# Gilgamesh666666/Point-cloud-registration-based-on-rotation-invariant-feature

Measured on AMD Instinct MI355X. Metric: point-clouds/sec (1024 pts, k=32) PPF+sph-vox forward, higher is better.
Workload: dtype f32; 1 GPU; sph-dg extractor forward: self-KNN k=32 + local PPF + sph-vox r=32^3 + sph-devox + descriptor; clouds_per_gpu=32, points=1024, k=32, resolution=32, channels=64, global_batch=32, parallelism=dp1 (clouds sharded, descriptor all-gather), schedule=6, steps_per_launch=200, distinct_batches=20

## Files before the change

### point-cloud-registration-based-on-rotation-invariant-feature_amd/csrc/knn_wsel.hip

```cpp
#include "knn_spatial.hpp"

namespace pcr {

template <int W>
constexpr int wsel_chunk() { return W == 8 ? 2 : 1; }
static inline bool wsel_narrow(int nblk, int b) { return (size_t)nblk * b * 8 > 4096; }
constexpr int kWselCap = 64;
constexpr int kWselTmax = 0x461C3FFF;

#define PCR_WSEL_VCC_STAGE(NAME, CTRL, LOW)                                        \
  __device__ inline unsigned NAME(unsigned x) {                                    \
    unsigned t;                                                                    \
    asm volatile("s_nop 1\n\t"                                                     \
                 "v_sub_co_u32_dpp %1, vcc, %0, %0 " CTRL " row_mask:0xf bank_mask:0xf\n\t" \
                 "s_xor_b32 vcc_lo, vcc_lo, " LOW "\n\t"                           \
                 "s_xor_b32 vcc_hi, vcc_hi, " LOW "\n\t"                           \
                 "v_cndmask_b32_dpp %0, %0, %0, vcc " CTRL " row_mask:0xf bank_mask:0xf" \
                 : "+v"(x), "=&v"(t)                                               \
                 :                                                                 \
                 : "vcc");                                                         \
    return x;                                                                      \
  }
PCR_WSEL_VCC_STAGE(wsel_x1, "quad_perm:[1,0,3,2]", "0x55555555")
PCR_WSEL_VCC_STAGE(wsel_x2, "quad_perm:[2,3,0,1]", "0x33333333")
PCR_WSEL_VCC_STAGE(wsel_m4, "quad_perm:[3,2,1,0]", "0x33333333")
#undef PCR_WSEL_VCC_STAGE
#define PCR_WSEL_MINMAX_STAGE(NAME, LO, HI, MLO, MHI)                              \
  __device__ inline unsigned NAME(unsigned x) {                                    \
    unsigned a;                                                                    \
    asm volatile("s_nop 1\n\t"                                                     \
                 "v_min_u32_dpp %0, %1, %1 " LO " " MLO "\n\t"                     \
                 "v_max_u32_dpp %0, %1, %1 " HI " " MHI                            \
                 : "=&v"(a)                                                        \
                 : "v"(x));                                                        \
    return a;                                                                      \
  }
PCR_WSEL_MINMAX_STAGE(wsel_m8, "row_half_mirror", "row_half_mirror",
                      "row_mask:0xf bank_mask:0x5", "row_mask:0xf bank_mask:0xa")
PCR_WSEL_MINMAX_STAGE(wsel_m16, "row_mirror", "row_mirror",
                      "row_mask:0xf bank_mask:0x3", "row_mask:0xf bank_mask:0xc")
PCR_WSEL_MINMAX_STAGE(wsel_x4, "row_shl:4", "row_shr:4",
                      "row_mask:0xf bank_mask:0x5", "row_mask:0xf bank_mask:0xa")
PCR_WSEL_MINMAX_STAGE(wsel_x8, "row_shl:8", "row_shr:8",
                      "row_mask:0xf bank_mask:0x3", "row_mask:0xf bank_mask:0xc")
#undef PCR_WSEL_MINMAX_STAGE
#define PCR_WSEL_ROW_STAGE(NAME, FETCH, RLO, RHI)                                  \
  __device__ inline unsigned NAME(unsigned x) {                                    \
    unsigned a, p;                                                                 \
    asm volatile("s_nop 1\n\t" FETCH                                               \
                 "s_nop 1\n\t"                                                     \
                 "v_min_u32_dpp %0, %1, %2 quad_perm:[0,1,2,3] row_mask:" RLO " bank_mask:0xf\n\t" \
                 "v_max_u32_dpp %0, %1, %2 quad_perm:[0,1,2,3] row_mask:" RHI " bank_mask:0xf" \
                 : "=&v"(a), "+v"(x), "=&v"(p)                                     \
                 :);                                                               \
    return a;                                                                      \
  }
PCR_WSEL_ROW_STAGE(wsel_x16,
                   "v_mov_b32_e32 %2, %1\n\t"
                   "s_nop 1\n\t"
                   "v_permlane16_swap_b32 %2, %2\n\t",
                   "0x5", "0xa")
PCR_WSEL_ROW_STAGE(wsel_m32,
                   "v_mov_b32_dpp %2, %1 row_mirror row_mask:0xf bank_mask:0xf\n\t"
                   "s_nop 1\n\t"
                   "v_permlane16_swap_b32 %2, %2\n\t",
                   "0x5", "0xa")
PCR_WSEL_ROW_STAGE(wsel_m64,
                   "v_mov_b32_dpp %2, %1 row_mirror row_mask:0xf bank_mask:0xf\n\t"
                   "s_nop 1\n\t"
                   "v_permlane16_swap_b32 %2, %2\n\t"
                   "s_nop 1\n\t"
                   "v_permlane32_swap_b32 %2, %2\n\t",
                   "0x3", "0xc")
#undef PCR_WSEL_ROW_STAGE

__device__ inline unsigned wsel_sort64(unsigned x) {
  x = wsel_x1(x);
  x = wsel_m4(x);
  x = wsel_x1(x);
  x = wsel_m8(x);
  x = wsel_x2(x);
  x = wsel_x1(x);
  x = wsel_m16(x);
  x = wsel_x4(x);
  x = wsel_x2(x);
  x = wsel_x1(x);
  x = wsel_m32(x);
  x = wsel_x8(x);
  x = wsel_x4(x);
  x = wsel_x2(x);
  x = wsel_x1(x);
  x = wsel_m64(x);
  x = wsel_x16(x);
  x = wsel_x8(x);
  x = wsel_x4(x);
  x = wsel_x2(x);
  x = wsel_x1(x);
  asm volatile("s_nop 1");
  return x;
}

__device__ inline unsigned long long wsel_sort64_exact(unsigned long long x, int lane) {
  for (int kk = 2; kk <= 64; kk <<= 1) {
    for (int jj = kk >> 1; jj > 0; jj >>= 1) {
      const int m = jj == (kk >> 1) ? kk - 1 : jj;
      const unsigned long long p = shfl_xor_u64(x, m);
      const bool lower = (lane & jj) == 0;
      x = lower ? (x < p ? x : p) : (x < p ? p : x);
    }
  }
  return x;
}

__device__ __attribute__((always_inline)) inline void wsel_append(unsigned long long m,
                                                                  unsigned addr, unsigned d,
                                                                  int lane, int r) {
  unsigned t, p;
  unsigned long long save;
  asm volatile("v_add_u32_e32 %0, %2, %1" : "=v"(p) : "v"(lane), "i"(64 * r));
  asm volatile(
      "s_mov_b64 %1, exec\n\t"
      "s_mov_b64 exec, %2\n\t"
      "v_mbcnt_lo_u32_b32 %0, %3, 0\n\t"
      "v_mbcnt_hi_u32_b32 %0, %4, %0\n\t"
      "v_lshl_add_u32 %0, %0, 2, %5\n\t"
      "ds_write2st64_b32 %0, %6, %7 offset1:1\n\t"
      "s_mov_b64 exec, %1"
      : "=&v"(t), "=&s"(save)
      : "s"(m), "s"((unsigned)m), "s"((unsigned)(m >> 32)), "s"(addr), "v"(d), "v"(p)
      : "memory");
}

template <int R, int W>
__global__ __launch_bounds__(W * 64) void knn_wsel_kernel(KnnSet s, int k) {
  constexpr int kWselWaves = W;
  constexpr int kWselChunk = wsel_chunk<W>();
  __shared__ unsigned kbuf_s[kWselWaves][2][kWselCap];
  __shared__ int tile_s[kBlk][kSortedK + 1];
  __shared__ int qnext_s;
  __shared__ __align__(16) float cx_s[R * kBlk], cy_s[R * kBlk], cz_s[R * kBlk];
  __shared__ __align__(16) int cj_s[R * kBlk];
  static_assert(sizeof(kbuf_s[0][0]) == 256, "wsel_append's offset");
  static_assert(sizeof(cx_s) % (64 * 16) == 0, "whole LDS-DMA pieces");
  const int b = blockIdx.y, qblk = blockIdx.x;
  const int wv = __builtin_amdgcn_readfirstlane(threadIdx.x >> 6);
  const int lane = threadIdx.x & 63;
  const size_t cb = (size_t)b * s.npad;
  lds_dma_copy<16>(cx_s, s.x + cb, 4 * s.npad);
  lds_dma_copy<16>(cy_s, s.y + cb, 4 * s.npad);
  lds_dma_copy<16>(cz_s, s.z + cb, 4 * s.npad);
  lds_dma_copy<16>(cj_s, s.j + cb, 4 * s.npad);
  if (threadIdx.x == 0) qnext_s = 0;
  wait_vmcnt<0>();
  __syncthreads();
  if (s.npad < R * kBlk) {
    for (int i = s.npad + threadIdx.x; i < R * kBlk; i += kWselWaves * kBlk) {
      cx_s[i] = cy_s[i] = cz_s[i] = __builtin_nanf("");
      cj_s[i] = -1;
    }
    __syncthreads();
  }
  typedef float pf2v __attribute__((ext_vector_type(2)));
  pf2v cx[R / 2], cy[R / 2], cz[R / 2];
#pragma unroll
  for (int h = 0; h < R / 2; h++) {
    const int p = 2 * h * kBlk + lane;
    cx[h] = pf2v{cx_s[p], cx_s[p + kBlk]};
    cy[h] = pf2v{cy_s[p], cy_s[p + kBlk]};
    cz[h] = pf2v{cz_s[p], cz_s[p + kBlk]};
  }
  const int pq = qblk * kBlk + lane;
  const float qxl = cx_s[pq], qyl = cy_s[pq], qzl = cz_s[pq];
  const int qjl = cj_s[pq];
  auto grab = [&]() {
    int v = 0;
    if (lane == 0)
      v = __hip_atomic_fetch_add(&qnext_s, kWselChunk, __ATOMIC_RELAXED, __HIP_MEMORY_SCOPE_WORKGROUP);
    return v;
  };
  int q0 = __builtin_amdgcn_readfirstlane(grab());
  int tb = kWselTmax;
  if (q0 < kBlk) {
    const float* bx = s.box + ((size_t)b * s.nblk + qblk) * 8;
    const float qx = readlane_f(qxl, q0), qy = readlane_f(qyl, q0), qz = readlane_f(qzl, q0);
    if (min(kBlk, s.n - qblk * kBlk) >= k) {
      const float u = box_ub(qx, qy, qz, bx);
      if (u < PCR_KNN_UNDEF) tb = (int)__float_as_uint(u);
    }
  }
  unsigned* kd = kbuf_s[wv][0];
  int* kj = (int*)kbuf_s[wv][1];
  const unsigned kd_addr =
      (unsigned)(uintptr_t)((__attribute__((address_space(3))) unsigned*)kd);
  const float tgt = 0.5f * (float)(k + kWselCap);
#pragma unroll 1
  for (int qi = q0; qi < kBlk;) {
    const int qj = __builtin_amdgcn_readlane(qjl, qi);
    if (qj < 0) {
      if (lane < kSortedK) tile_s[qi][lane] = 0;
      if (++qi % kWselChunk == 0) qi = __builtin_amdgcn_readfirstlane(grab());
      continue;
    }
    const float qx = readlane_f(qxl, qi), qy = readlane_f(qyl, qi), qz = readlane_f(qzl, qi);
    const pf2v qx2 = {qx, qx}, qy2 = {qy, qy}, qz2 = {qz, qz};
    unsigned db[R];
#pragma unroll
    for (int h = 0; h < R / 2; h++) {
      const pf2v a = qx2 - cx[h], bq = qy2 - cy[h], c = qz2 - cz[h];
      pf2v d = a * a;
      d = __builtin_elementwise_fma(bq, bq, d);
      d = __builtin_elementwise_fma(c, c, d);
      db[2 * h] = __float_as_uint(d[0]);
      db[2 * h + 1] = __float_as_uint(d[1]);
    }
    constexpr bool kKeep = R <= 16;
    unsigned long long msk[kKeep ? R : 1];
    auto count_le = [&](int bits) {
      int pc[4] = {0, 0, 0, 0};
#pragma unroll
      for (int r = 0; r < R; r++) {
        const unsigned long long m = __ballot(db[r] <= (unsigned)bits);
        if (kKeep) msk[kKeep ? r : 0] = m;
        pc[r & 3] += __popcll(m);
      }
      return (pc[0] + pc[1]) + (pc[2] + pc[3]);
    };
    int lo = -1, hi = 0x7F800000, cnt_lo = 0, cnt = 0;
    bool exact = false;
#pragma unroll 1
    for (int pass = 0;; pass++) {
      cnt = count_le(tb);
      if (cnt >= k && cnt <= kWselCap) break;
      if (cnt < k) {
        lo = tb;
        cnt_lo = cnt;
        if (tb >= kWselTmax) break;
      } else {
        hi = tb;
      }
      if (hi - lo <= 1) {
        exact = true;
        break;
      }
      int nb;
      if (pass < 3) {
        const float f = __uint_as_float((unsigned)tb) *
                        __builtin_amdgcn_exp2f(0.6666667f * __builtin_amdgcn_logf(
                                                                tgt * __builtin_amdgcn_rcpf((float)max(cnt, 1))));
        nb = f < 1e30f ? (int)__float_as_uint(f) : kWselTmax;
      } else {
        nb = lo + ((hi - lo) >> 1);
      }
      nb = min(nb, kWselTmax);
      if (nb <= lo || nb >= hi) nb = lo + ((hi - lo) >> 1);
      tb = __builtin_amdgcn_readfirstlane(nb);
    }
    int ntake;
    if (!exact) {
      unsigned addr = kd_addr;
#pragma unroll
      for (int r = 0; r < R; r++) {
        const unsigned long long m = kKeep ? msk[kKeep ? r : 0] : __ballot(db[r] <= (unsigned)tb);
        if (m != 0ull) {
          wsel_append(m, addr, db[r], lane, r);
          addr += 4u * (unsigned)__popcll(m);
        }
      }
      ntake = cnt;
    } else {
      const int need = k - cnt_lo;
      auto cj = [&](int r) { return cj_s[64 * r + lane]; };
      int jl = -1, jh = s.n - 1;
#pragma unroll 1
      while (jh - jl > 1) {
        const int jm = jl + ((jh - jl) >> 1);
        int c = 0;
#pragma unroll
        for (int r = 0; r < R; r++) c += __popcll(__ballot(db[r] == (unsigned)hi && cj(r) <= jm));
        if (c >= need) jh = jm;
        else jl = jm;
      }
      unsigned addr = kd_addr;
#pragma unroll
      for (int r = 0; r < R; r++) {
        const unsigned long long m =
            __ballot(db[r] < (unsigned)hi || (db[r] == (unsigned)hi && cj(r) <= jh));
        if (m != 0ull) {
          wsel_append(m, addr, db[r], lane, r);
          addr += 4u * (unsigned)__popcll(m);
        }
      }
      ntake = k;
    }
    const unsigned dl = lane < ntake ? kd[lane] : 0xFFFFFFFFu;
    unsigned key = lane < ntake ? ((dl >> 6) << 6) | (unsigned)lane : 0x7FFFFFFFu;
    key = wsel_sort64(key);
    const unsigned nxt = (unsigned)__builtin_amdgcn_mov_dpp((int)key, 0x130, 0xF, 0xF, false);
    const bool tie = lane < k && lane + 1 < ntake && (key >> 6) == (nxt >> 6);
    const bool slow = __any(tie);
    if (!slow) {
      const int jo = lane < ntake ? cj_s[kj[key & 63u]] : 0;
      if (lane < k) tile_s[qi][lane] = jo;
    } else {
      unsigned long long skey = ~0ull;
      if (lane < ntake) skey = ((unsigned long long)kd[lane] << 32) | (unsigned)cj_s[kj[lane]];
      skey = wsel_sort64_exact(skey, lane);
      if (lane < k) tile_s[qi][lane] = lane < ntake ? (int)(unsigned)(skey & 0xFFFFFFFFull) : 0;
    }
    __atomic_signal_fence(__ATOMIC_SEQ_CST);
    if (++qi % kWselChunk == 0) qi = __builtin_amdgcn_readfirstlane(grab());
  }
  __syncthreads();
  for (int sl = wv; sl < k; sl += kWselWaves)
    s.sidx[((size_t)b * kSortedK + sl) * s.npad + (size_t)qblk * kBlk + lane] = tile_s[lane][sl];
}

void launch_wsel(const KnnSet& s, int b, int k, hipStream_t st) {
  if (wsel_narrow(s.nblk, b))
    hipLaunchKernelGGL((knn_wsel_kernel<16, 8>), dim3(s.nblk, b), dim3(8 * 64), 0, st, s, k);
  else
    hipLaunchKernelGGL((knn_wsel_kernel<16, 12>), dim3(s.nblk, b), dim3(12 * 64), 0, st, s, k);
}

}
```

Before: 474,400 point-clouds/sec.

## Search KNN threshold on per-lane minima before a full exact-count fallback

The radius-threshold search in the wave-select KNN now runs on each lane's minimum distance (a single ballot per pass) rather than counting every candidate register on each pass. Each step uses a precomputed log-log order-statistic table held in lanes to jump the threshold. Candidates are then appended once with a capacity guard, and the earlier full count/bisect path runs only when the resulting count falls outside [k, cap]. This trims ballot and popcount work per search pass, but adds an extra append pass and a fallback path whenever the lane-minimum estimate misses.

Result: no change. 471,400 point-clouds/sec (-0.6%).

```diff
diff --git a/point-cloud-registration-based-on-rotation-invariant-feature_amd/csrc/knn_wsel.hip b/point-cloud-registration-based-on-rotation-invariant-feature_amd/csrc/knn_wsel.hip
--- a/point-cloud-registration-based-on-rotation-invariant-feature_amd/csrc/knn_wsel.hip
+++ b/point-cloud-registration-based-on-rotation-invariant-feature_amd/csrc/knn_wsel.hip
@@ -7,6 +7,9 @@
 static inline bool wsel_narrow(int nblk, int b) { return (size_t)nblk * b * 8 > 4096; }
 constexpr int kWselCap = 64;
 constexpr int kWselTmax = 0x461C3FFF;
+constexpr int kWselLaneWin = 4;
+constexpr int kWselLaneEst = 5;
+constexpr float kWselLaneInv = 1.0f / 64.5f;
 
 #define PCR_WSEL_VCC_STAGE(NAME, CTRL, LOW)                                        \
   __device__ inline unsigned NAME(unsigned x) {                                    \
@@ -193,6 +196,11 @@
   const unsigned kd_addr =
       (unsigned)(uintptr_t)((__attribute__((address_space(3))) unsigned*)kd);
   const float tgt = 0.5f * (float)(k + kWselCap);
+  auto lane_g = [](float m) {
+    return (int)(5592405.0f * __log2f(-__log2f(1.0f - kWselLaneInv * m)));
+  };
+  const int gtab = lane_g((float)(lane + 1));
+  const int gtgt = __builtin_amdgcn_readfirstlane(lane_g((float)k + 0.5f * (float)kWselLaneWin));
 #pragma unroll 1
   for (int qi = q0; qi < kBlk;) {
     const int qj = __builtin_amdgcn_readlane(qjl, qi);
@@ -213,84 +221,119 @@
       db[2 * h] = __float_as_uint(d[0]);
       db[2 * h + 1] = __float_as_uint(d[1]);
     }
-    constexpr bool kKeep = R <= 16;
-    unsigned long long msk[kKeep ? R : 1];
-    auto count_le = [&](int bits) {
-      int pc[4] = {0, 0, 0, 0};
-#pragma unroll
-      for (int r = 0; r < R; r++) {
-        const unsigned long long m = __ballot(db[r] <= (unsigned)bits);
-        if (kKeep) msk[kKeep ? r : 0] = m;
-        pc[r & 3] += __popcll(m);
-      }
-      return (pc[0] + pc[1]) + (pc[2] + pc[3]);
-    };
-    int lo = -1, hi = 0x7F800000, cnt_lo = 0, cnt = 0;
-    bool exact = false;
+    unsigned lm = min(db[0], db[1]);
+#pragma unroll
+    for (int r = 2; r < R; r += 2) lm = min(min(lm, db[r]), db[r + 1]);
+    int lo = -1, hi = 0x7F800000;
 #pragma unroll 1
     for (int pass = 0;; pass++) {
-      cnt = count_le(tb);
-      if (cnt >= k && cnt <= kWselCap) break;
-      if (cnt < k) {
+      const int m = __popcll(__ballot(lm <= (unsigned)tb));
+      if ((unsigned)(m - k) <= (unsigned)kWselLaneWin) break;
+      if (m < k) {
         lo = tb;
-        cnt_lo = cnt;
         if (tb >= kWselTmax) break;
       } else {
         hi = tb;
       }
       if (hi - lo <= 1) {
-        exact = true;
+        tb = hi;
         break;
       }
-      int nb;
-      if (pass < 3) {
-        const float f = __uint_as_float((unsigned)tb) *
-                        __builtin_amdgcn_exp2f(0.6666667f * __builtin_amdgcn_logf(
-                                                                tgt * __builtin_amdgcn_rcpf((float)max(cnt, 1))));
-        nb = f < 1e30f ? (int)__float_as_uint(f) : kWselTmax;
+      int nb = tb + (gtgt - __builtin_amdgcn_readlane(gtab, max(m, 1) - 1));
+      if (pass >= kWselLaneEst || nb <= lo || nb >= hi) nb = lo + ((hi - lo) >> 1);
+      tb = min(nb, kWselTmax);
+    }
+    const unsigned kd_end = kd_addr + 4u * kWselCap;
+    int cnt;
+    {
+      unsigned addr = kd_addr;
+#pragma unroll
+      for (int r = 0; r < R; r++) {
+        const unsigned long long m = __ballot(db[r] <= (unsigned)tb);
+        if (m != 0ull) {
+          const unsigned na = addr + 4u * (unsigned)__popcll(m);
+          if (na <= kd_end) wsel_append(m, addr, db[r], lane, r);
+          addr = na;
+        }
+      }
+      cnt = (int)((addr - kd_addr) >> 2);
+    }
+    int ntake = cnt;
+    if (!((cnt >= k && cnt <= kWselCap) || (cnt < k && tb >= kWselTmax))) {
+      auto count_le = [&](int bits) {
+        int pc[4] = {0, 0, 0, 0};
+#pragma unroll
+        for (int r = 0; r < R; r++) pc[r & 3] += __popcll(__ballot(db[r] <= (unsigned)bits));
+        return (pc[0] + pc[1]) + (pc[2] + pc[3]);
+      };
+      int cnt_lo = 0;
+      bool exact = false;
+      lo = -1;
+      hi = 0x7F800000;
+#pragma unroll 1
+      for (int pass = 0;; pass++) {
+        if (cnt < k) {
+          lo = tb;
+          cnt_lo = cnt;
+          if (tb >= kWselTmax) break;
+        } else {
+          hi = tb;
+        }
+        if (hi - lo <= 1) {
+          exact = true;
+          break;
+        }
+        int nb;
+        if (pass < 3) {
+          const float f = __uint_as_float((unsigned)tb) *
+                          __builtin_amdgcn_exp2f(0.6666667f * __builtin_amdgcn_logf(
+                                                                  tgt * __builtin_amdgcn_rcpf((float)max(cnt, 1))));
+          nb = f < 1e30f ? (int)__float_as_uint(f) : kWselTmax;
+        } else {
+          nb = lo + ((hi - lo) >> 1);
+        }
+        nb = min(nb, kWselTmax);
+        if (nb <= lo || nb >= hi) nb = lo + ((hi - lo) >> 1);
+        tb = __builtin_amdgcn_readfirstlane(nb);
+        cnt = count_le(tb);
+        if (cnt >= k && cnt <= kWselCap) break;
+      }
+      if (!exact) {
+        unsigned addr = kd_addr;
+#pragma unroll
+        for (int r = 0; r < R; r++) {
+          const unsigned long long m = __ballot(db[r] <= (unsigned)tb);
+          if (m != 0ull) {
+            wsel_append(m, addr, db[r], lane, r);
+            addr += 4u * (unsigned)__popcll(m);
+          }
+        }
+        ntake = cnt;
       } else {
-        nb = lo + ((hi - lo) >> 1);
-      }
-      nb = min(nb, kWselTmax);
-      if (nb <= lo || nb >= hi) nb = lo + ((hi - lo) >> 1);
-      tb = __builtin_amdgcn_readfirstlane(nb);
-    }
-    int ntake;
-    if (!exact) {
-      unsigned addr = kd_addr;
-#pragma unroll
-      for (int r = 0; r < R; r++) {
-        const unsigned long long m = kKeep ? msk[kKeep ? r : 0] : __ballot(db[r] <= (unsigned)tb);
-        if (m != 0ull) {
-          wsel_append(m, addr, db[r], lane, r);
-          addr += 4u * (unsigned)__popcll(m);
-        }
-      }
-      ntake = cnt;
-    } else {
-      const int need = k - cnt_lo;
-      auto cj = [&](int r) { return cj_s[64 * r + lane]; };
-      int jl = -1, jh = s.n - 1;
+        const int need = k - cnt_lo;
+        auto cj = [&](int r) { return cj_s[64 * r + lane]; };
+        int jl = -1, jh = s.n - 1;
 #pragma unroll 1
-      while (jh - jl > 1) {
-        const int jm = jl + ((jh - jl) >> 1);
-        int c = 0;
-#pragma unroll
-        for (int r = 0; r < R; r++) c += __popcll(__ballot(db[r] == (unsigned)hi && cj(r) <= jm));
-        if (c >= need) jh = jm;
-        else jl = jm;
-      }
-      unsigned addr = kd_addr;
-#pragma unroll
-      for (int r = 0; r < R; r++) {
-        const unsigned long long m =
-            __ballot(db[r] < (unsigned)hi || (db[r] == (unsigned)hi && cj(r) <= jh));
-        if (m != 0ull) {
-          wsel_append(m, addr, db[r], lane, r);
-          addr += 4u * (unsigned)__popcll(m);
-        }
-      }
-      ntake = k;
+        while (jh - jl > 1) {
+          const int jm = jl + ((jh - jl) >> 1);
+          int c = 0;
+#pragma unroll
+          for (int r = 0; r < R; r++) c += __popcll(__ballot(db[r] == (unsigned)hi && cj(r) <= jm));
+          if (c >= need) jh = jm;
+          else jl = jm;
+        }
+        unsigned addr = kd_addr;
+#pragma unroll
+        for (int r = 0; r < R; r++) {
+          const unsigned long long m =
+              __ballot(db[r] < (unsigned)hi || (db[r] == (unsigned)hi && cj(r) <= jh));
+          if (m != 0ull) {
+            wsel_append(m, addr, db[r], lane, r);
+            addr += 4u * (unsigned)__popcll(m);
+          }
+        }
+        ntake = k;
+      }
     }
     const unsigned dl = lane < ntake ? kd[lane] : 0xFFFFFFFFu;
     unsigned key = lane < ntake ? ((dl >> 6) << 6) | (unsigned)lane : 0x7FFFFFFFu;
```
